# Tommachilez/improving-learned-index

Measured on AMD Instinct MI355X. Metric: docs/sec encoded + queries/sec@top-1000, MS MARCO passage, 1/2/4/8 MI355X, higher is better.
Workload: dtype bf16x3

## Files before the change

improving-learned-index_amd/csrc/enc_attn.hip:

```cpp
#include <hip/hip_runtime.h>

#include <algorithm>
#include <cstdlib>
#include <type_traits>

#include "di_common.h"
#include "enc_common.h"

namespace di {

constexpr int ATT_D = 64;
constexpr int QT = 4;

__host__ __device__ __forceinline__ int vt_base(int doc, int tok0) { return 32 * (doc + (tok0 >> 5)); }

template <typename T>
struct AttnOps;
template <>
struct AttnOps<bf16> {
    static constexpr int KC = 32;
    static constexpr int EPC = 8;
};
template <>
struct AttnOps<float> {
    static constexpr int KC = 16;
    static constexpr int EPC = 4;
};

__device__ __forceinline__ void mma_chunk(const uint4 &a, const uint4 &b, f32x4 &acc, bf16) {
    bf16x8 av, bv;
    __builtin_memcpy(&av, &a, 16);
    __builtin_memcpy(&bv, &b, 16);
    acc = __builtin_amdgcn_mfma_f32_16x16x32_bf16(av, bv, acc, 0, 0, 0);
}
__device__ __forceinline__ void mma_chunk(const uint4 &a, const uint4 &b, f32x4 &acc, float) {
    acc = __builtin_amdgcn_mfma_f32_16x16x4f32(__uint_as_float(a.x), __uint_as_float(b.x), acc,
                                               0, 0, 0);
    acc = __builtin_amdgcn_mfma_f32_16x16x4f32(__uint_as_float(a.y), __uint_as_float(b.y), acc,
                                               0, 0, 0);
    acc = __builtin_amdgcn_mfma_f32_16x16x4f32(__uint_as_float(a.z), __uint_as_float(b.z), acc,
                                               0, 0, 0);
    acc = __builtin_amdgcn_mfma_f32_16x16x4f32(__uint_as_float(a.w), __uint_as_float(b.w), acc,
                                               0, 0, 0);
}

template <typename T>
__global__ void __launch_bounds__(64)
attention_kernel(const T *__restrict__ qk, const T *__restrict__ vt,
                 const int32_t *__restrict__ cu_seqlens, int H, int ld_v, int n_qb, int n_heads,
                 int n_pairs, T *__restrict__ ctx, bf16 *__restrict__ ctx_split) {
    constexpr int KC = AttnOps<T>::KC, EPC = AttnOps<T>::EPC;
    constexpr int NCH = ATT_D / KC;
    const int id = blockIdx.x, x = id & 7, j = id >> 3;
    const int pair = (j / n_qb) * 8 + x;
    const int qb = j % n_qb;
    if (pair >= n_pairs) return;
    const int doc = pair / n_heads, h = pair % n_heads;
    const int lane = threadIdx.x;
    const int g = lane >> 4, c = lane & 15;
    const int tok0 = cu_seqlens[doc], n = cu_seqlens[doc + 1] - tok0;
// ... 112 lines not shown
                    acc = __builtin_amdgcn_mfma_f32_16x16x4f32(__uint_as_float(a0.w), s[0][3], acc, 0, 0, 0);
                    acc = __builtin_amdgcn_mfma_f32_16x16x4f32(__uint_as_float(a1.x), s[1][0], acc, 0, 0, 0);
                    acc = __builtin_amdgcn_mfma_f32_16x16x4f32(__uint_as_float(a1.y), s[1][1], acc, 0, 0, 0);
                    acc = __builtin_amdgcn_mfma_f32_16x16x4f32(__uint_as_float(a1.z), s[1][2], acc, 0, 0, 0);
                    acc = __builtin_amdgcn_mfma_f32_16x16x4f32(__uint_as_float(a1.w), s[1][3], acc, 0, 0, 0);
                    o[qt][dt] = acc;
                }
            }
        }
    }
#pragma unroll
    for (int qt = 0; qt < QT; ++qt) {
        float l = lsum[qt];
        l += __shfl_xor(l, 16, 64);
        l += __shfl_xor(l, 32, 64);
        const float inv = 1.0f / l;
        const int q = q_base + 16 * qt + c;
        if (q < n && ctx_split) {
            bf16 *out = ctx_split + (int64_t)(tok0 + q) * 2 * H;
#pragma unroll
            for (int dt = 0; dt < 4; ++dt) {
                bf16x4 hv, lv;
#pragma unroll
                for (int r = 0; r < 4; ++r) hv[r] = split_hi(o[qt][dt][r] * inv), lv[r] = split_lo(o[qt][dt][r] * inv);
                const int64_t sc0 = split_col(h * ATT_D + dt * 16 + 4 * g);
                *reinterpret_cast<bf16x4 *>(out + sc0) = hv;
                *reinterpret_cast<bf16x4 *>(out + sc0 + 32) = lv;
            }
        } else if (q < n) {
            T *out = ctx + (int64_t)(tok0 + q) * H + h * ATT_D + 4 * g;
#pragma unroll
            for (int dt = 0; dt < 4; ++dt) {
                if constexpr (sizeof(T) == 2) {
                    bf16x4 v;
#pragma unroll
                    for (int r = 0; r < 4; ++r) v[r] = (bf16)(o[qt][dt][r] * inv);
                    *reinterpret_cast<bf16x4 *>(out + dt * 16) = v;
                } else {
                    *reinterpret_cast<float4 *>(out + dt * 16) =
                        make_float4(o[qt][dt][0] * inv, o[qt][dt][1] * inv, o[qt][dt][2] * inv,
                                    o[qt][dt][3] * inv);
                }
            }
        }
    }
}

constexpr int AX_WAVES = 8, AX_QT = 2;
__device__ __forceinline__ int ax_swz(int r) { return ((r & 3) << 1) | (r & 8); }
constexpr int AX_KC = 64, AX_IMG = AX_KC * 256, AX_LDS = 4 * AX_IMG;
constexpr int AX_QTB = 4096;
constexpr int ax_lds(int nw, int qtn, int kc = AX_KC) { return 4 * kc * 256 + nw * qtn * AX_QTB; }

template <bool BAL, bool LAZY, bool PIPE = false, int NW = AX_WAVES, int QTN = AX_QT,
          int KC = AX_KC>
__global__ void __launch_bounds__(64 * NW) __attribute__((amdgpu_waves_per_eu(2)))
attention_x3_kernel(const bf16 *__restrict__ qkv, const int32_t *__restrict__ cu_seqlens, int H,
                    int n_heads, int n_pairs, bf16 *__restrict__ ctx_split,
                    const int32_t *__restrict__ qsel, const int32_t *__restrict__ cu_qsel,
                    int abl) {
    extern __shared__ __attribute__((aligned(16))) unsigned char lds[];
    typedef __attribute__((address_space(3))) void lds_void;
    const int tid = threadIdx.x, lane = tid & 63;
    const int wave = __builtin_amdgcn_readfirstlane(tid >> 6);
    const int g = lane >> 4, c = lane & 15;
    const int64_t ld = 6 * (int64_t)H;
    const uint32_t lds_base =
        (uint32_t)(uintptr_t)((__attribute__((address_space(3))) unsigned char *)lds);
    const float sc = 0.125f * 1.4426950408889634f;
    constexpr int PASS_Q = NW * QTN * 16;
    static_assert(QTN == 2 || QTN == 3, "two or three query tiles per wave");
    constexpr int IMG = KC * 256, KVL = 4 * IMG;

    struct Unit {
        int pair, pass, tok0, n, h, q0, nq;
    };
    auto make_unit = [&](int pr, int pass, Unit &u) {
        const int doc = pr / n_heads;
        u.pair = pr;
        u.pass = pass;
        u.h = pr % n_heads;
        u.tok0 = cu_seqlens[doc];
        u.n = cu_seqlens[doc + 1] - u.tok0;
        u.q0 = qsel ? cu_qsel[doc] : u.tok0;
        u.nq = qsel ? cu_qsel[doc + 1] - u.q0 : u.n;
    };
    auto next_unit = [&](const Unit &u, Unit &nu) {
        if ((u.pass + 1) * PASS_Q < u.nq && !(abl & 16)) {
            nu = u;
            nu.pass = u.pass + 1;
            return true;
        }
        for (int pr = u.pair + (int)gridDim.x; pr < n_pairs; pr += (int)gridDim.x) {
            make_unit(pr, 0, nu);
            if (nu.n > 0 && nu.nq > 0) return true;
        }
        return false;
    };
    constexpr int RPW = KC / NW;
    const int sr = RPW * wave + (lane >> 4);
    auto stage = [&](const Unit &u, int ci, int b) {
        const bf16 *kg = qkv + split_col(H + u.h * ATT_D);
        const bf16 *vg = qkv + split_col(2 * H + u.h * ATT_D);
#pragma unroll
        for (int pc = 0; pc < RPW / 4; ++pc) {
            const int rl = sr + 4 * pc;
            const int row = u.tok0 + min(ci * KC + rl, u.n - 1);
            const int j = (lane & 15) ^ ax_swz(rl);
            const int dst = b * IMG + (RPW * wave + 4 * pc) * 256;
            __builtin_amdgcn_global_load_lds((const void *)(kg + row * ld + j * 8),
                                             (lds_void *)(lds + dst), 16, 0, 0);
            __builtin_amdgcn_global_load_lds((const void *)(vg + row * ld + j * 8),
                                             (lds_void *)(lds + 2 * IMG + dst), 16, 0, 0);
        }
    };
    auto qtile = [&](int qt) { return BAL ? 16 * (wave + NW * qt) : wave * (QTN * 16) + 16 * qt; };
    auto dma_q = [&](const Unit &u) {
        const bf16 *qbase = qkv + split_col(u.h * ATT_D) + 8 * g;
#pragma unroll
        for (int qt = 0; qt < QTN; ++qt) {
            const int qi = min(u.pass * PASS_Q + qtile(qt) + c, u.nq - 1);
            const int qloc = qsel ? min(max(qsel[u.q0 + qi], 0), u.n - 1) : qi;
            const int qrow = u.tok0 + qloc;
#pragma unroll
            for (int ch = 0; ch < 2; ++ch) {
                const bf16 *src = qbase + qrow * ld + ch * 64;
                const int dst = KVL + wave * (QTN * AX_QTB) + (qt * 2 + ch) * 2048;
                __builtin_amdgcn_global_load_lds((const void *)src, (lds_void *)(lds + dst), 16, 0, 0);
                __builtin_amdgcn_global_load_lds((const void *)(src + 32),
                                                 (lds_void *)(lds + dst + 1024), 16, 0, 0);
            }
        }
    };
    constexpr int AX_HALF = 1024;
    uint32_t ka[2][2];
#pragma unroll
    for (int ch = 0; ch < 2; ++ch)
#pragma unroll
        for (int pt = 0; pt < 2; ++pt) {
            const int r = 8 * (c >> 2) + (c & 3), j = ch * 8 + pt * 4 + g;
            ka[ch][pt] = lds_base + r * 256 + ((j ^ ax_swz(r)) << 4);
        }
    uint32_t va[4][2];
#pragma unroll
    for (int dt = 0; dt < 4; ++dt)
#pragma unroll
        for (int pt = 0; pt < 2; ++pt) {
            const int q = c >> 2, pp = c & 3;
            const int r = 8 * g + q;
            const int j = (dt >> 1) * 8 + pt * 4 + 2 * (dt & 1) + (pp >> 1);
            va[dt][pt] = lds_base + 2 * IMG + r * 256 + ((j ^ ax_swz(r)) << 4) + 8 * (pp & 1);
        }

    Unit cu;
    {
        int pr = blockIdx.x;
        for (; pr < n_pairs; pr += (int)gridDim.x) {
            make_unit(pr, 0, cu);
            if (cu.n > 0 && cu.nq > 0) break;
        }
        if (pr >= n_pairs) return;
    }
    bf16x8 qh[QTN][2], ql[QTN][2];
    const uint32_t qa = lds_base + KVL + wave * (QTN * AX_QTB) + lane * 16;
    auto read_q = [&]() {
        uint4 q4[8];
        asm volatile(
            "ds_read_b128 %0, %8 offset:0"
            "\n\tds_read_b128 %1, %8 offset:1024"
            "\n\tds_read_b128 %2, %8 offset:2048"
            "\n\tds_read_b128 %3, %8 offset:3072"
            "\n\tds_read_b128 %4, %8 offset:4096"
            "\n\tds_read_b128 %5, %8 offset:5120"
            "\n\tds_read_b128 %6, %8 offset:6144"
            "\n\tds_read_b128 %7, %8 offset:7168"
            "\n\ts_waitcnt lgkmcnt(0)"
            : "=&v"(q4[0]), "=&v"(q4[1]), "=&v"(q4[2]), "=&v"(q4[3]), "=&v"(q4[4]),
              "=&v"(q4[5]), "=&v"(q4[6]), "=&v"(q4[7])
            : "v"(qa)
            : "memory");
#pragma unroll
        for (int qt = 0; qt < 2; ++qt)
#pragma unroll
            for (int ch = 0; ch < 2; ++ch) {
                __builtin_memcpy(&qh[qt][ch], &q4[(qt * 2 + ch) * 2], 16);
                __builtin_memcpy(&ql[qt][ch], &q4[(qt * 2 + ch) * 2 + 1], 16);
            }
        if constexpr (QTN == 3) {
            uint4 q5[4];
            asm volatile(
                "ds_read_b128 %0, %4 offset:8192"
                "\n\tds_read_b128 %1, %4 offset:9216"
                "\n\tds_read_b128 %2, %4 offset:10240"
                "\n\tds_read_b128 %3, %4 offset:11264"
                "\n\ts_waitcnt lgkmcnt(0)"
                : "=&v"(q5[0]), "=&v"(q5[1]), "=&v"(q5[2]), "=&v"(q5[3])
                : "v"(qa)
                : "memory");
#pragma unroll
            for (int ch = 0; ch < 2; ++ch) {
                __builtin_memcpy(&qh[2][ch], &q5[ch * 2], 16);
                __builtin_memcpy(&ql[2][ch], &q5[ch * 2 + 1], 16);
            }
        }
    };
    stage(cu, 0, 0);
    dma_q(cu);
    int b = 0;
    for (;;) {
        const int n = cu.n, h = cu.h, q0 = cu.q0, nq = cu.nq;
        const int q_pass = cu.pass * PASS_Q;
        const bool has_q = q_pass + qtile(0) < nq;
        const bool two = BAL ? q_pass + qtile(1) < nq : has_q;
        const bool three = QTN == 3 && (BAL ? q_pass + qtile(2) < nq : has_q);
// ... 352 lines not shown
                            vfr[dt][p == 1], p == 2 ? pl[qt] : ph[qt], o[qt][dt], 0, 0, 0);
            }
            }
            };
            chunk(nqt_outer);
        };
        const int n_whole = n / KC;
        int ci = 0;
        for (; ci < n_whole; ++ci, b ^= 1) one_chunk(ci, std::true_type{});
        if (ci < n_chunks) {
            one_chunk(ci, std::false_type{});
            b ^= 1;
        }
        };
        if (!has_q) {
            for (int ci = 0; ci < n_chunks; ++ci, b ^= 1)
                if (ci > 0) stage_step(ci);
        } else if (three) {
            if constexpr (QTN == 3) chunk_loop(std::integral_constant<int, 3>{});
        } else if (two) {
            chunk_loop(std::integral_constant<int, 2>{});
        } else {
            chunk_loop(std::integral_constant<int, 1>{});
        }
        if (has_q) {
#pragma unroll
            for (int qt = 0; qt < QTN; ++qt) {
                float l = lsum[qt];
                l += __shfl_xor(l, 16, 64);
                l += __shfl_xor(l, 32, 64);
                const float inv = 1.0f / l;
                const int q = q_pass + qtile(qt) + c;
                if (q < nq) {
                    bf16 *out = ctx_split + (int64_t)(q0 + q) * 2 * H;
#pragma unroll
                    for (int dt = 0; dt < 4; ++dt) {
                        bf16x4 hv, lv;
#pragma unroll
                        for (int r = 0; r < 4; ++r) {
                            const float y = o[qt][dt][r] * inv;
                            hv[r] = split_hi(y);
                            lv[r] = split_lo(y);
                        }
                        const int64_t sc0 = split_col(h * ATT_D + dt * 16 + 4 * g);
                        *reinterpret_cast<bf16x4 *>(out + sc0) = hv;
                        *reinterpret_cast<bf16x4 *>(out + sc0 + 32) = lv;
                    }
                }
            }
        }
        if (!more) break;
        cu = nu;
    }
#undef AX_READ_K
#undef AX_READ_VW
#undef AX_SEL
}

void launch_attention_x3(const bf16 *qkv, const int32_t *cu_seqlens, int n_docs, int H,
                         bf16 *ctx_split, hipStream_t s, const int32_t *qsel,
                         const int32_t *cu_qsel) {
    DI_REQUIRE(H % ATT_D == 0, DI_EINVAL, "hidden %d is not a multiple of the head dim 64", H);
    if (n_docs == 0) return;
    const int n_heads = H / ATT_D;
    const int64_t n_pairs = (int64_t)n_docs * n_heads;
    DI_REQUIRE(n_pairs < (1ll << 31), DI_ERANGE, "attention grid too large");
    static const int variant = [] {
        const char *e = getenv("DI_ATTN_X3");
        return e ? atoi(e) & 252 : 92;
    }();

    static const int abl = [] {
        const char *e = getenv("DI_ATTN_X3_ABLATE");
        return e ? atoi(e) : 0;
    }();
#define AX_LAUNCH(BL, LZ, PP, NW, QN, KC)                                                      \
    do {                                                                                       \
        DI_HIP(hipFuncSetAttribute((const void *)attention_x3_kernel<BL, LZ, PP, NW, QN, KC>,  \
                                   hipFuncAttributeMaxDynamicSharedMemorySize,                 \
                                   ax_lds(NW, QN, KC)));                                       \
        hipLaunchKernelGGL((attention_x3_kernel<BL, LZ, PP, NW, QN, KC>),                      \
                           dim3((int)std::min<int64_t>(                                        \
                               n_pairs, (int64_t)n_cu() * (160 * 1024 / ax_lds(NW, QN, KC)))), \
                           dim3(64 * NW), ax_lds(NW, QN, KC), s, qkv, cu_seqlens, H, n_heads,  \
                           (int)n_pairs, ctx_split, qsel, cu_qsel, abl);                       \
    } while (0)
    static const int pruned_variant = [] {
        const char *e = getenv("DI_ATTN_X3_PRUNED");
        return e ? atoi(e) : 1;
    }();
    if (qsel && pruned_variant == 1 && variant == 92) {
        AX_LAUNCH(true, true, true, 4, 3, 32);
        check_launch("attention_x3");
        return;
    }
    switch (variant) {
    case 12: AX_LAUNCH(true, true, false, AX_WAVES, AX_QT, AX_KC); break;
    case 28: AX_LAUNCH(true, true, true, AX_WAVES, AX_QT, AX_KC); break;
    case 60: AX_LAUNCH(true, true, true, 4, AX_QT, AX_KC); break;
    case 92: AX_LAUNCH(true, true, true, AX_WAVES, 3, AX_KC); break;
    case 220: AX_LAUNCH(true, true, true, 4, 3, 32); break;
    default: AX_LAUNCH(false, false, false, AX_WAVES, AX_QT, AX_KC); break;
    }
#undef AX_LAUNCH
    check_launch("attention_x3");
}

__device__ __forceinline__ bool softmax_need(const f32x4 (&s)[2], float lim) {
    bool need = false;
#pragma unroll
    for (int t = 0; t < 2; ++t)
#pragma unroll
        for (int r = 0; r < 4; ++r) need |= s[t][r] > lim;
    return need;
}
__device__ __forceinline__ void softmax_rescale(const f32x4 (&s)[2], float lim, float &m,
                                                float &msc, f32x4 (&o)[4], f32x4 &l) {
    constexpr float sc = 0.125f * 1.4426950408889634f;
    float cmax = fmaxf(fmaxf(fmaxf(s[0][0], s[0][1]), fmaxf(s[0][2], s[0][3])),
                       fmaxf(fmaxf(s[1][0], s[1][1]), fmaxf(s[1][2], s[1][3])));
    const auto p16 = __builtin_amdgcn_permlane16_swap(__float_as_uint(cmax),
                                                      __float_as_uint(cmax), false, false);
    cmax = fmaxf(__uint_as_float(p16[0]), __uint_as_float(p16[1]));
    const auto p32 = __builtin_amdgcn_permlane32_swap(__float_as_uint(cmax),
                                                      __float_as_uint(cmax), false, false);
    cmax = fmaxf(__uint_as_float(p32[0]), __uint_as_float(p32[1]));
    const float m_new = cmax > lim ? fmaxf(m, cmax) : m;
    const float alpha = exp2f((m - m_new) * sc);
    m = m_new;
    msc = m_new * sc;
    l *= alpha;
#pragma unroll
    for (int dt = 0; dt < 4; ++dt) o[dt] *= alpha;
}
__device__ __forceinline__ void softmax_p(const f32x4 (&s)[2], float msc, bf16x8 &pb) {
    constexpr float sc = 0.125f * 1.4426950408889634f;
#pragma unroll
    for (int r = 0; r < 4; ++r) {
        pb[r] = (bf16)__builtin_amdgcn_exp2f(fmaf(s[0][r], sc, -msc));
        pb[4 + r] = (bf16)__builtin_amdgcn_exp2f(fmaf(s[1][r], sc, -msc));
    }
}

constexpr int ATT3_WAVES = 8;
template <bool DB>
struct Att3 {
    static constexpr int ROWS = DB ? 320 : 512;
    static constexpr int BUF = 2 * ROWS * 128;
    static constexpr int LDS = DB ? 2 * BUF : BUF;
};

__device__ __forceinline__ int att3_swz(int r) { return (r & 7) ^ ((r >> 1) & 4); }

template <int K, int N, class F>
__device__ __forceinline__ void att3_chunks(F &f) {
    if constexpr (K < N) {
        if (f(std::integral_constant<int, K>{})) return;
        att3_chunks<K + 1, N>(f);
// ... 432 lines not shown
```

improving-learned-index_amd/csrc/enc_handle.h:

```cpp
#pragma once

#include <memory>
#include <vector>

#include "di_common.h"
#include "pair_order.h"

namespace di {

struct Layer {
    DevBuf w_qkv, b_qkv, w_o, b_o, ln1_g, ln1_b, w_i, b_i, w_out, b_out, ln2_g, ln2_b;
    DevBuf s_qkv, c_qkv, s_i, c_i;
};

struct PairRun {
    const int32_t *tt, *ct;
    const int64_t *cu_sq;
    int max_len;
};

}

struct di_encoder {
    di_encoder_cfg cfg{};
    int device = 0;
    hipStream_t stream = nullptr;
    bool own_stream = false;
    size_t esz = 2;
    bool split = false;
    di::DevBuf word, pos, type0, emb_g, emb_b, head_w;
    float head_b = 0.f;
    std::vector<std::unique_ptr<di::Layer>> layers;
    di::DevBuf X, qk, vt, vcol, ctx, pre, X1, Hff, impact, ids, cu, tt, cut, err;
    bool folded = false;
    di::DevBuf stats1, stats2, head_wg;
    di::DevBuf rln1, rln2;
    float head_sw = 0.f, head_cw = 0.f;
    int64_t cap_tokens = 0;
    int64_t cap_rows = 0;
    int cap_docs = 0;
    int ld_v = 0;
    bool has_pair = false;
    di::DevBuf pair_w, Mx, uv, cu_sq, cup;
    float pair_w0 = 0.f, pair_b = 0.f;
    const di::PairRun *pair_run = nullptr;
    di::DevBuf ent_single, ent_pair, ent_pos;
    di::PairOrderWs order;
    di::DevBuf pinfo;
    di::Timer timer;
};

namespace di {

void ensure_workspace(di_encoder *e, int64_t M, int n_docs, int64_t n_terms);

}
```

improving-learned-index_amd/csrc/encoder.hip:

```cpp
#include <hip/hip_runtime.h>

#include <cstdlib>
#include <type_traits>

#include <cmath>
#include <cstring>
#include <memory>
#include <string>
#include <unordered_map>
#include <vector>

#include "di_common.h"
#include "enc_common.h"
#include "enc_handle.h"

namespace di {

template <typename T>
void launch_gemm(int epi, const GemmArgs &g, hipStream_t s);
template <typename T>
void launch_attention(const T *qk, const T *vt, const int32_t *cu_seqlens, int n_docs,
                      int max_len, int H, int ld_v, T *ctx, hipStream_t s,
                      bf16 *ctx_split = nullptr);
void launch_gemm256(int epi, const GemmArgs &g, hipStream_t s);
void launch_attention_x3(const bf16 *qkv, const int32_t *cu_seqlens, int n_docs, int H,
                         bf16 *ctx_split, hipStream_t s, const int32_t *qsel = nullptr,
                         const int32_t *cu_qsel = nullptr);
void launch_scatter_term_rows(const bf16 *Xg, const int32_t *cu_seq, const int32_t *cu_terms,
                              const int32_t *term_tok, int n_docs, int W, int64_t ld, bf16 *X,
                              hipStream_t s);
void launch_embed_ln_split(const int32_t *ids, const int32_t *cu, int n_docs, int M, int H,
                           const float *word, const float *pos, const float *type0,
                           const float *gamma, const float *beta, float eps, int pos_offset,
                           int vocab, int max_pos, bf16 *out, int32_t *err, hipStream_t s);
void launch_ln_split(const float *pre, int M, int H, const float *gamma, const float *beta,
                     float eps, bf16 *out, const float *head_w, float head_b, int act,
                     float *impact, hipStream_t s);
template <typename T>
void launch_embed_ln(const int32_t *ids, const int32_t *cu, int n_docs, int M, int H,
                     const T *word, const T *pos, const T *type0, const float *gamma,
                     const float *beta, float eps, int pos_offset, int vocab, int max_pos, T *out,
                     int32_t *err, hipStream_t s);
template <typename T>
void launch_ln(const T *pre, int M, int H, const float *gamma, const float *beta, float eps,
               T *out, const float *head_w, float head_b, int act, float *impact, hipStream_t s);
void launch_vt_cols(const int32_t *cu, int n_docs, int M, int32_t *vcol, hipStream_t s);
bool attention_v3_ok(int max_len, int H);
void launch_head_from_stats(const float4 *st, int ld, int n_part, int M, int H, float eps,
                            float sw, float cw, int act, float *impact, hipStream_t s);
void launch_row_ln(const float4 *st, int ld, int n_part, int M, int H, float eps, float2 *out,
                   hipStream_t s);
int gemm_stats_cols();
void launch_attention_v3(const bf16 *qkv, const int32_t *cu_seqlens, int n_docs, int max_len,
                         int H, bf16 *ctx, hipStream_t s, const int32_t *qsel = nullptr,
                         const int32_t *cu_qsel = nullptr);
void launch_gather_term_rows(const bf16 *X, const float2 *rl, const int32_t *cu_seq,
                             const int32_t *cu_terms, const int32_t *term_tok, int n_docs, int H,
                             bf16 *Xg, float2 *rlg, hipStream_t s);
int vt_ld(int64_t M, int n_docs);
void launch_gather_terms(const float *impact, const int32_t *cu_seq, const int32_t *cu_terms,
                         int n_docs, const int32_t *term_tok, int n_terms, int do_round,
                         float *out, int32_t *err, hipStream_t s);

size_t pair_attn_lds_bytes(int max_len);
void launch_pair_prep(const int32_t *cu_seq, const int32_t *cu_terms, const int32_t *term_tok,
                      const int64_t *cu_pairs, int n_docs, int64_t n_terms, int64_t n_pairs,
                      int max_len, int64_t *cu_sq, int32_t *err, hipStream_t s);
void launch_pair_attn(const void *qk, bool split, const int32_t *cu_seq, const int32_t *cu_terms,
                      const int32_t *term_tok, const int64_t *cu_sq, int n_docs, int max_len,
                      int H, float *Mx, const int32_t *err, hipStream_t s);
void launch_pair_score(const void *src, int src_mode, const int32_t *cu_seq,
                       const int32_t *cu_terms, const int32_t *term_tok,
                       const int64_t *cu_pairs, const int64_t *cu_sq, int n_docs,
                       int64_t n_terms, int64_t n_pairs, int H, const float *gamma,
                       const float *beta, float eps, const float *w, float w0, float bias,
                       const float *Mx, float2 *uv, int do_round, float *out_pair,
                       float *out_attn, const int32_t *err, hipStream_t s);

}

// ... 122 lines not shown
            uint16_t *o = &h[(size_t)(r * 2 * K)];
            for (int k = 0; k < K; ++k) {
                const float w = p->at(i * K + k);
                const uint16_t hi = f32_to_bf16_bits(w);
                const uint16_t lo = f32_to_bf16_bits(w - bf16_bits_to_f32(hi));
                o[split_col(k)] = hi;
                o[split_col(k) + 32] = lo;
            }
        }
    }
    dst.reserve(h.size() * 2);
    DI_HIP(hipMemcpy(dst.p, h.data(), h.size() * 2, hipMemcpyHostToDevice));
}

}

void di::ensure_workspace(di_encoder *e, int64_t M, int n_docs, int64_t n_terms) {
    const int H = e->cfg.hidden, F = e->cfg.intermediate;
    if (M > e->cap_tokens || n_docs > e->cap_docs) {
        int64_t cap = std::max<int64_t>(std::max<int64_t>(M, e->cap_tokens), 256);
        const int capd = std::max(std::max(n_docs, e->cap_docs), 16);
        const size_t es = e->esz;
        const int64_t capr = (cap + 255) / 256 * 256;
        e->X.reserve(capr * H * es);
        e->X1.reserve(capr * H * es);
        e->ctx.reserve(capr * H * es);
        e->qk.reserve(cap * 3 * H * es);
        e->Hff.reserve(capr * std::max(F, H) * es);
        e->pre.reserve(cap * H * es);
        e->impact.reserve(cap * 4);
        e->ids.reserve(cap * 4);
        const size_t vt_bytes = e->split ? 0 : (size_t)H * vt_ld(cap, capd) * es;
        if (!e->split) e->vcol.reserve(cap * 4);
        if (vt_bytes > e->vt.bytes) {
            e->vt.reserve(vt_bytes);
            DI_HIP(hipMemset(e->vt.p, 0, vt_bytes));
        }
        if (e->folded) {
            const size_t sb = (size_t)(H / 128) * capr * 16;
            e->stats1.reserve(sb);
            e->stats2.reserve(sb);
            e->rln1.reserve((size_t)capr * 8);
            e->rln2.reserve((size_t)capr * 8);
        }
        e->cap_tokens = cap;
        e->cap_rows = capr;
        e->cap_docs = capd;
    }
    e->ld_v = vt_ld(M, n_docs);
    e->cu.reserve((size_t)(n_docs + 1) * 4);
    e->cut.reserve((size_t)(n_docs + 1) * 4);
    e->tt.reserve((size_t)std::max<int64_t>(n_terms, 1) * 4);
    e->err.reserve(16);
    if (e->has_pair) {
        e->uv.reserve((size_t)std::max<int64_t>(n_terms, 1) * 8);
        e->cu_sq.reserve((size_t)(n_docs + 1) * 8);
        e->cup.reserve((size_t)(n_docs + 1) * 8);
        e->ent_single.reserve((size_t)std::max<int64_t>(n_terms, 1) * 4);
        e->ent_pos.reserve((size_t)std::max<int64_t>(n_terms, 1) * 4);
        e->order.reserve_docs(n_docs);
    }
}

namespace {

void pair_attn_layer(di_encoder *e, const int32_t *d_cu, int n_docs, bool timing,
                     hipStream_t s) {
    const PairRun *r = e->pair_run;
    if (!r) return;
    TimedLaunch tl(e->timer, timing, "pair_attn", s);
    launch_pair_attn(e->qk.p, e->split, d_cu, r->ct, r->tt, r->cu_sq, n_docs, r->max_len,
                     e->cfg.hidden, e->Mx.as<float>(), e->err.as<int32_t>(), s);
}

template <typename T>
void forward(di_encoder *e, const int32_t *d_ids, const int32_t *d_cu, int n_docs, int64_t M,
             int max_len, bool timing, hipStream_t s) {
    const auto &c = e->cfg;
    const int H = c.hidden, F = c.intermediate;
    const int pos_offset = (c.variant == DI_VARIANT_XLMR) ? c.pad_id + 1 : 0;
    T *X = e->X.as<T>(), *X1 = e->X1.as<T>();
    {
        TimedLaunch tl(e->timer, timing, "embed_ln", s);
        launch_embed_ln<T>(d_ids, d_cu, n_docs, (int)M, H, e->word.as<T>(), e->pos.as<T>(),
                           e->type0.as<T>(), e->emb_g.as<float>(), e->emb_b.as<float>(),
                           c.layer_norm_eps, pos_offset, c.vocab_size, c.max_positions, X,
                           e->err.as<int32_t>(), s);
    }
    const bool use_v3 = std::is_same<T, bf16>::value && attention_v3_ok(max_len, H);
    if (!use_v3) launch_vt_cols(d_cu, n_docs, (int)M, e->vcol.as<int32_t>(), s);
    for (size_t l = 0; l < e->layers.size(); ++l) {
        Layer &L = *e->layers[l];
        const bool last = l + 1 == e->layers.size();
        GemmArgs g{};
        g.M = (int)M;
        g.a_rows = e->cap_rows;
        g.hidden = H;
        if (use_v3) {
            g.A = X;
            g.B = L.w_qkv.p;
            g.bias = L.b_qkv.as<float>();
            g.out = e->qk.p;
            g.N = 3 * H;
            g.K = H;
            g.ld_out = 3 * H;
            {
// ... 147 lines not shown
            TimedLaunch tl(e->timer, timing, "gather_rows", s);
            Xr = e->Hff.as<bf16>();
            launch_gather_term_rows(X, P ? rl2 : nullptr, d_cu, d_ct, d_tt, n_docs, H * W2, Xr,
                                    rl1, s);
            rl2r = rl1;
        };
        const bool qc = prune && sp;
        if (qc) gather_rows();
        GemmArgs g = base();
        g.A = X;
        g.B = L.w_qkv.p;
        g.bias = L.b_qkv.as<float>();
        g.out = e->qk.p;
        g.N = 3 * H;
        g.K = H;
        g.ld_out = 3 * H * W2;
        if (P) {
            g.row_ln = rl2;
            g.col_s = L.s_qkv.as<float>();
            g.col_c = L.c_qkv.as<float>();
        }
        {
            TimedLaunch tl(e->timer, timing, "gemm_qkv", s);
            if (!qc) {
                gemm(P ? EPI_FOLD : EPI_BIAS, g);
            } else {
                GemmArgs gk = g;
                gk.B = static_cast<const bf16 *>(L.w_qkv.p) + (int64_t)H * 2 * H;
                gk.bias = L.b_qkv.as<float>() + H;
                if (P) {
                    gk.col_s = L.s_qkv.as<float>() + H;
                    gk.col_c = L.c_qkv.as<float>() + H;
                }
                gk.out = e->qk.as<bf16>() + 2 * H;
                gk.N = 2 * H;
                gemm(P ? EPI_FOLD : EPI_BIAS, gk);
                GemmArgs gq = g;
                gq.A = Xr;
                gq.M = (int)n_terms;
                gq.N = H;
                gq.out = e->ctx.p;
                gq.ld_out = 2 * H;
                gq.row_ln = P ? rl1 : nullptr;
                gemm(P ? EPI_FOLD : EPI_BIAS, gq);
                launch_scatter_term_rows(e->ctx.as<bf16>(), d_cu, d_ct, d_tt, n_docs, 2 * H,
                                         6 * (int64_t)H, e->qk.as<bf16>(), s);
            }
        }
        if (sp) pair_attn_layer(e, d_cu, n_docs, timing, s);
        {
            TimedLaunch tl(e->timer, timing, "attention", s);
            if (sp)
                launch_attention_x3(e->qk.as<bf16>(), d_cu, n_docs, H, e->ctx.as<bf16>(), s,
                                    prune ? d_tt : nullptr, prune ? d_ct : nullptr);
            else
                launch_attention_v3(e->qk.as<bf16>(), d_cu, n_docs, max_len, H,
                                    e->ctx.as<bf16>(), s, prune ? d_tt : nullptr,
                                    prune ? d_ct : nullptr);
        }
        if (prune && !qc) gather_rows();
        auto base_r = [&]() {
            GemmArgs gr = base();
            gr.M = (int)Mr;
            return gr;
        };
        g = base_r();
        g.A = e->ctx.p;
        g.B = L.w_o.p;
        g.bias = L.b_o.as<float>();
        g.resid = Xr;
        g.out = X1;
        g.N = H;
        g.K = H;
        g.ld_out = H * W2;
        g.stats_out = st1;
        if (P) {
            g.row_ln = rl2r;
            g.res_gamma = P->ln2_g.as<float>();
            g.res_beta = P->ln2_b.as<float>();
        }
        {
            TimedLaunch tl(e->timer, timing, "gemm_o", s);
            gemm(EPI_RESID_STATS, g);
        }
        {
            TimedLaunch tl(e->timer, timing, "row_ln", s);
            launch_row_ln(st1, ld, n_part, (int)Mr, H, c.layer_norm_eps, rl1, s);
        }
        g = base_r();
        g.A = X1;
        g.B = L.w_i.p;
        g.out = e->Hff.p;
        g.N = F;
        g.K = H;
        g.ld_out = F * W2;
        g.row_ln = rl1;
        g.col_s = L.s_i.as<float>();
        g.col_c = L.c_i.as<float>();
        {
            TimedLaunch tl(e->timer, timing, "gemm_ffn1", s);
            gemm(EPI_FOLD_GELU, g);
        }
        g = base_r();
        g.A = e->Hff.p;
        g.B = L.w_out.p;
        g.bias = L.b_out.as<float>();
        g.resid = X1;
// ... 21 lines not shown
        launch_head_from_stats(st2, ld, n_part, (int)(d_tt ? n_terms : M), H, c.layer_norm_eps,
                               e->head_sw,
                               e->head_cw, c.activation, e->impact.as<float>(), s);
    }
}

void forward_split(di_encoder *e, const int32_t *d_ids, const int32_t *d_cu, int n_docs,
                   int64_t M, int max_len, bool timing, hipStream_t s,
                   const int32_t *d_tt = nullptr, const int32_t *d_ct = nullptr,
                   int64_t n_terms = 0) {
    const auto &c = e->cfg;
    const int H = c.hidden, F = c.intermediate;
    const int pos_offset = (c.variant == DI_VARIANT_XLMR) ? c.pad_id + 1 : 0;
    bf16 *X = e->X.as<bf16>(), *X1 = e->X1.as<bf16>(), *ctx = e->ctx.as<bf16>();
    float *pre = e->pre.as<float>();
    {
        TimedLaunch tl(e->timer, timing, "embed_ln", s);
        launch_embed_ln_split(d_ids, d_cu, n_docs, (int)M, H, e->word.as<float>(),
                              e->pos.as<float>(), e->type0.as<float>(), e->emb_g.as<float>(),
                              e->emb_b.as<float>(), c.layer_norm_eps, pos_offset, c.vocab_size,
                              c.max_positions, X, e->err.as<int32_t>(), s);
    }
    auto base = [&]() {
        GemmArgs g{};
        g.M = (int)M;
        g.a_rows = e->cap_rows;
        g.hidden = H;
        g.tune_gm = 8;
        g.split = 1;
        return g;
    };
    for (size_t l = 0; l < e->layers.size(); ++l) {
        Layer &L = *e->layers[l];
        const bool last = l + 1 == e->layers.size();
        GemmArgs g = base();
        g.A = X;
        g.B = L.w_qkv.p;
        g.bias = L.b_qkv.as<float>();
        g.out = e->qk.p;
        g.N = 3 * H;
        g.K = H;
        g.ld_out = 6 * H;
        {
            TimedLaunch tl(e->timer, timing, "gemm_qkv", s);
            launch_gemm256(EPI_BIAS, g, s);
        }
        const bool prune = last && d_tt != nullptr;
        const int64_t Mr = prune ? n_terms : M;
        bf16 *Xr = X;
        pair_attn_layer(e, d_cu, n_docs, timing, s);
        {
            TimedLaunch tl(e->timer, timing, "attention", s);
            launch_attention_x3(e->qk.as<bf16>(), d_cu, n_docs, H, ctx, s,
                                prune ? d_tt : nullptr, prune ? d_ct : nullptr);
        }
        if (prune) {
            TimedLaunch tl(e->timer, timing, "gather_rows", s);
            Xr = e->Hff.as<bf16>();
            launch_gather_term_rows(X, nullptr, d_cu, d_ct, d_tt, n_docs, 2 * H, Xr, nullptr, s);
        }
        auto base_r = [&]() {
            GemmArgs gr = base();
            gr.M = (int)Mr;
            return gr;
        };
        g = base_r();
        g.A = ctx;
        g.B = L.w_o.p;
        g.bias = L.b_o.as<float>();
        g.resid = Xr;
        g.out = pre;
        g.N = H;
        g.K = H;
        g.ld_out = H;
        {
            TimedLaunch tl(e->timer, timing, "gemm_o", s);
            launch_gemm256(EPI_BIAS_RESID, g, s);
        }
        {
            TimedLaunch tl(e->timer, timing, "ln", s);
            launch_ln_split(pre, (int)Mr, H, L.ln1_g.as<float>(), L.ln1_b.as<float>(),
                            c.layer_norm_eps, X1, nullptr, 0.f, c.activation, nullptr, s);
        }
        g = base_r();
        g.A = X1;
        g.B = L.w_i.p;
        g.bias = L.b_i.as<float>();
        g.out = e->Hff.p;
        g.N = F;
        g.K = H;
        g.ld_out = 2 * F;
        {
            TimedLaunch tl(e->timer, timing, "gemm_ffn1", s);
            launch_gemm256(EPI_BIAS_GELU, g, s);
        }
        g = base_r();
        g.A = e->Hff.p;
        g.B = L.w_out.p;
        g.bias = L.b_out.as<float>();
        g.resid = X1;
        g.out = pre;
        g.N = H;
        g.K = F;
        g.ld_out = H;
        g.tune_gm = 4;
        {
            TimedLaunch tl(e->timer, timing, "gemm_ffn2", s);
// ... 65 lines not shown
                mx_need += T * T;
            }
            n_pairs = pc->cu_pairs[n_docs];
        }
    } else if (pc) {
        DI_REQUIRE(n_terms >= 0 && n_terms <= n_tokens && n_pairs >= 0, DI_EINVAL,
                   "n_terms=%lld n_pairs=%lld", (long long)n_terms, (long long)n_pairs);
        mx_need = n_terms * std::min<int64_t>(n_terms, max_len);
    }
    DI_REQUIRE(n_tokens >= 0 && n_tokens < (1ll << 31), DI_ERANGE, "n_tokens=%lld",
               (long long)n_tokens);
    DI_REQUIRE(max_len <= e->cfg.max_positions, DI_ERANGE,
               "a document has %d tokens > max_positions %d", max_len,
               e->cfg.max_positions);
    if (pc && pc->n_terms_out) *pc->n_terms_out = n_terms, *pc->n_pairs_out = n_pairs;
    if (n_docs == 0) return;
    ensure_workspace(e, n_tokens, n_docs, n_terms);
    float *out_pair = pc ? pc->out_pair : nullptr;
    if (pc && pc->dev_out) {
        e->ent_pair.reserve((size_t)std::max<int64_t>(n_pairs, 1) * 4);
        out = e->ent_single.as<float>();
        out_pair = e->ent_pair.as<float>();
    }
    const int32_t *d_ids = stage_in(tok_ids, (size_t)n_tokens, dev, e->ids, s);
    const int32_t *d_cu = stage_in(cu_seqlens, (size_t)n_docs + 1, dev, e->cu, s);
    DI_HIP(hipMemsetAsync(e->err.p, 0, 4, s));
    const int32_t *d_tt = nullptr, *d_cut = nullptr;
    if (!token_out) {
        d_tt = stage_in(term_tok, (size_t)n_terms, dev, e->tt, s);
        d_cut = stage_in(cu_terms, (size_t)n_docs + 1, dev, e->cut, s);
    }
    PairRun run{};
    struct RunScope {
        di_encoder *e;
        ~RunScope() { e->pair_run = nullptr; }
    } run_scope{e};
    const int64_t *d_cup = nullptr;
    if (pc) {
        DI_REQUIRE(pair_attn_lds_bytes(max_len) <= 160 * 1024, DI_ERANGE,
                   "pairwise: a document of %d tokens exceeds the LDS panel", max_len);
        DI_REQUIRE(mx_need <= (1ll << 32), DI_ERANGE,
                   "pairwise: %lld term-pair slots in one batch (limit 2^32)",
                   (long long)mx_need);
        e->Mx.reserve((size_t)std::max<int64_t>(mx_need, 1) * 4);
        d_cup = stage_in(pc->cu_pairs, (size_t)n_docs + 1, dev, e->cup, s);
        {
            TimedLaunch tl(e->timer, timing, "pair_prep", s);
            if (mx_need) DI_HIP(hipMemsetAsync(e->Mx.p, 0, (size_t)mx_need * 4, s));
            launch_pair_prep(d_cu, d_cut, d_tt, d_cup, n_docs, n_terms, n_pairs, max_len,
                             e->cu_sq.as<int64_t>(), e->err.as<int32_t>(), s);
        }
        run = PairRun{d_tt, d_cut, e->cu_sq.as<int64_t>(), max_len};
        if (n_pairs > 0) e->pair_run = &run;
    }
    const bool prune = !token_out && (e->split || (e->esz == 2 && e->folded)) &&
                       n_terms <= n_tokens;
    if (n_tokens > 0) {
        if (e->split && !e->folded)
            forward_split(e, d_ids, d_cu, n_docs, n_tokens, max_len, timing, s,
                          prune ? d_tt : nullptr, prune ? d_cut : nullptr, n_terms);
        else if (e->split)
            forward_folded(e, d_ids, d_cu, n_docs, n_tokens, max_len, timing, s,
                           prune ? d_tt : nullptr, prune ? d_cut : nullptr, n_terms);
        else if (e->esz == 2)
            if (e->folded)
                forward_folded(e, d_ids, d_cu, n_docs, n_tokens, max_len, timing, s,
                               prune ? d_tt : nullptr, prune ? d_cut : nullptr, n_terms);
            else
                forward<bf16>(e, d_ids, d_cu, n_docs, n_tokens, max_len, timing, s);
        else
            forward<float>(e, d_ids, d_cu, n_docs, n_tokens, max_len, timing, s);
    }
    float *d_out = out;
    DevBuf tmp;
    if (token_out) {
        if (dev)
            DI_HIP(hipMemcpyAsync(out, e->impact.p, (size_t)n_tokens * 4,
                                  hipMemcpyDeviceToDevice, s));
        else
            DI_HIP(hipMemcpyAsync(out, e->impact.p, (size_t)n_tokens * 4,
                                  hipMemcpyDeviceToHost, s));
    } else {
        if (!dev_out) {
            tmp.reserve((size_t)std::max<int64_t>(n_terms, 1) * 4);
            d_out = tmp.as<float>();
        }
        {
            TimedLaunch tl(e->timer, timing, "gather_terms", s);
            launch_gather_terms(e->impact.as<float>(), d_cu, d_cut, n_docs, d_tt,
                                (int)n_terms,
                                ((flags & DI_F_ROUND3) ? 1 : 0) | (prune && n_tokens > 0 ? 2 : 0),
                                d_out, e->err.as<int32_t>(), s);
        }
        if (!dev_out && n_terms)
            DI_HIP(hipMemcpyAsync(out, d_out, (size_t)n_terms * 4, hipMemcpyDeviceToHost,
                                  s));
    }
    DevBuf tmp_pair, tmp_attn;
    if (pc && n_pairs > 0) {
        float *d_pair = out_pair, *d_attn = pc->out_attn;
        if (!dev_out) {
            tmp_pair.reserve((size_t)n_pairs * 4);
            d_pair = tmp_pair.as<float>();
            if (pc->out_attn) {
                tmp_attn.reserve((size_t)n_pairs * 4);
                d_attn = tmp_attn.as<float>();
// ... 321 lines not shown
```

Measured before the change: 12270.

## Sort docs by length for attention scheduling and split long/short launches

Adds a single-block GPU kernel that counting-sorts documents by descending length and writes boundaries for long (>192 tokens) and short groups. The attention_x3 kernel now walks this order in a serpentine block assignment, which balances per-block work and shrinks tail imbalance. By default it also runs two launches, a large 8-wave configuration for long docs and a smaller 4-wave/KC=32 one for short docs. The cost is an extra serial sort kernel per batch and a second attention launch. The grid size now uses the queried LDS-per-CU instead of a hardcoded 160KB.

```diff
diff --git a/improving-learned-index_amd/csrc/enc_attn.hip b/improving-learned-index_amd/csrc/enc_attn.hip
--- a/improving-learned-index_amd/csrc/enc_attn.hip
+++ b/improving-learned-index_amd/csrc/enc_attn.hip
@@ -1,11 +1,14 @@
 #include <hip/hip_runtime.h>
 
 #include <algorithm>
+#include <atomic>
 #include <cstdlib>
 #include <type_traits>
+#include <vector>
 
 #include "di_common.h"
 #include "enc_common.h"
+#include "enc_handle.h"
 
 namespace di {
 
@@ -224,18 +227,28 @@
 constexpr int AX_QTB = 4096;
 constexpr int ax_lds(int nw, int qtn, int kc = AX_KC) { return 4 * kc * 256 + nw * qtn * AX_QTB; }
 
+#ifdef DI_ATTN_STAMP
+__device__ unsigned long long ax_stamp[2][1024];
+#endif
+
 template <bool BAL, bool LAZY, bool PIPE = false, int NW = AX_WAVES, int QTN = AX_QT,
           int KC = AX_KC>
 __global__ void __launch_bounds__(64 * NW) __attribute__((amdgpu_waves_per_eu(2)))
 attention_x3_kernel(const bf16 *__restrict__ qkv, const int32_t *__restrict__ cu_seqlens, int H,
                     int n_heads, int n_pairs, bf16 *__restrict__ ctx_split,
                     const int32_t *__restrict__ qsel, const int32_t *__restrict__ cu_qsel,
+                    const int32_t *__restrict__ q_order, const int32_t *__restrict__ q_range,
                     int abl) {
     extern __shared__ __attribute__((aligned(16))) unsigned char lds[];
     typedef __attribute__((address_space(3))) void lds_void;
     const int tid = threadIdx.x, lane = tid & 63;
     const int wave = __builtin_amdgcn_readfirstlane(tid >> 6);
     const int g = lane >> 4, c = lane & 15;
+#ifdef DI_ATTN_STAMP
+    if (lane == 0)
+        atomicMin(&ax_stamp[0][blockIdx.x], (unsigned long long)__builtin_amdgcn_s_memrealtime());
+    __builtin_amdgcn_s_waitcnt(0xC07F);
+#endif
     const int64_t ld = 6 * (int64_t)H;
     const uint32_t lds_base =
         (uint32_t)(uintptr_t)((__attribute__((address_space(3))) unsigned char *)lds);
@@ -245,17 +258,24 @@
     constexpr int IMG = KC * 256, KVL = 4 * IMG;
 
     struct Unit {
-        int pair, pass, tok0, n, h, q0, nq;
+        int r, pass, tok0, n, h, q0, nq;
     };
-    auto make_unit = [&](int pr, int pass, Unit &u) {
-        const int doc = pr / n_heads;
-        u.pair = pr;
-        u.pass = pass;
-        u.h = pr % n_heads;
+    const int q_lo = q_order ? q_range[0] : 0;
+    const int n_units = q_order ? (q_range[1] - q_lo) * n_heads : n_pairs;
+    auto make_unit = [&](int r, Unit &u) {
+        const int gs = (int)gridDim.x, bx = (int)blockIdx.x;
+        const int64_t i = (int64_t)r * gs + ((q_order && (r & 1)) ? gs - 1 - bx : bx);
+        if (i >= n_units) return false;
+        const int di = (int)i / n_heads;
+        const int doc = q_order ? q_order[q_lo + di] : di;
+        u.r = r;
+        u.pass = 0;
+        u.h = (int)i - di * n_heads;
         u.tok0 = cu_seqlens[doc];
         u.n = cu_seqlens[doc + 1] - u.tok0;
         u.q0 = qsel ? cu_qsel[doc] : u.tok0;
         u.nq = qsel ? cu_qsel[doc + 1] - u.q0 : u.n;
+        return true;
     };
     auto next_unit = [&](const Unit &u, Unit &nu) {
         if ((u.pass + 1) * PASS_Q < u.nq && !(abl & 16)) {
@@ -263,10 +283,8 @@
             nu.pass = u.pass + 1;
             return true;
         }
-        for (int pr = u.pair + (int)gridDim.x; pr < n_pairs; pr += (int)gridDim.x) {
-            make_unit(pr, 0, nu);
+        for (int r = u.r + 1; make_unit(r, nu); ++r)
             if (nu.n > 0 && nu.nq > 0) return true;
-        }
         return false;
     };
     constexpr int RPW = KC / NW;
@@ -325,13 +343,9 @@
         }
 
     Unit cu;
-    {
-        int pr = blockIdx.x;
-        for (; pr < n_pairs; pr += (int)gridDim.x) {
-            make_unit(pr, 0, cu);
-            if (cu.n > 0 && cu.nq > 0) break;
-        }
-        if (pr >= n_pairs) return;
+    for (int r = 0;; ++r) {
+        if (!make_unit(r, cu)) return;
+        if (cu.n > 0 && cu.nq > 0) break;
     }
     bf16x8 qh[QTN][2], ql[QTN][2];
     const uint32_t qa = lds_base + KVL + wave * (QTN * AX_QTB) + lane * 16;
@@ -790,14 +804,169 @@
         if (!more) break;
         cu = nu;
     }
+#ifdef DI_ATTN_STAMP
+    if (lane == 0)
+        atomicMax(&ax_stamp[1][blockIdx.x], (unsigned long long)__builtin_amdgcn_s_memrealtime());
+#endif
 #undef AX_READ_K
 #undef AX_READ_VW
 #undef AX_SEL
 }
 
+constexpr int AQ_THREADS = 1024, AQ_TILE = 4096;
+__global__ void __launch_bounds__(AQ_THREADS)
+attn_order_kernel(const int32_t *__restrict__ cu_seqlens, int n_docs, int max_len, int long_len,
+                  int32_t *__restrict__ order, int32_t *__restrict__ ctl) {
+    extern __shared__ int32_t aq_lds[];
+    int32_t *start = aq_lds, *tile = aq_lds + (max_len + 1);
+    const int tid = threadIdx.x;
+    auto len_of = [&](int d) {
+        return min(max(cu_seqlens[d + 1] - cu_seqlens[d], 0), max_len);
+    };
+    for (int b = tid; b <= max_len; b += AQ_THREADS) start[b] = 0;
+    __syncthreads();
+    for (int d = tid; d < n_docs; d += AQ_THREADS) atomicAdd(&start[len_of(d)], 1);
+    __syncthreads();
+    if (tid == 0) {
+        int acc = 0, n_long = 0;
+        for (int b = max_len; b >= 0; --b) {
+            const int cnt = start[b];
+            start[b] = acc;
+            acc += cnt;
+            if (b == long_len + 1) n_long = acc;
+        }
+        ctl[0] = 0;
+        ctl[1] = n_long;
+        ctl[2] = n_docs;
+        ctl[3] = 0;
+        ctl[4] = n_docs;
+    }
+    __syncthreads();
+    for (int t0 = 0; t0 < n_docs; t0 += AQ_TILE) {
+        const int nt = min(AQ_TILE, n_docs - t0);
+        for (int i = tid; i < nt; i += AQ_THREADS) tile[i] = len_of(t0 + i);
+        __syncthreads();
+        for (int b = tid; b <= max_len; b += AQ_THREADS) {
+            int pos = start[b];
+            for (int i = 0; i < nt; ++i)
+                if (tile[i] == b) order[pos++] = t0 + i;
+            start[b] = pos;
+        }
+        __syncthreads();
+    }
+}
+
+bool attn_order_ok(int max_positions) {
+    return max_positions >= 0 && (size_t)(max_positions + 1 + AQ_TILE) * 4 <= 64 * 1024;
+}
+
+void launch_attn_order(const int32_t *cu_seqlens, int n_docs, int max_positions, int32_t *order,
+                       int32_t *ctl, hipStream_t s) {
+    DI_REQUIRE(attn_order_ok(max_positions), DI_ERANGE, "attention order: max_positions %d",
+               max_positions);
+    hipLaunchKernelGGL(attn_order_kernel, dim3(1), dim3(AQ_THREADS),
+                       (size_t)(max_positions + 1 + AQ_TILE) * 4, s, cu_seqlens, n_docs,
+                       max_positions, AQ_LONG_LEN, order, ctl);
+    check_launch("attn_order");
+}
+
+int attn_queue_mode() {
+    static const int mode = [] {
+        const char *e = getenv("DI_ATTN_X3_QUEUE");
+        return e ? atoi(e) : 2;
+    }();
+    return mode;
+}
+
+namespace {
+
+void ax_lds_limits(int &per_cu, int &per_wg) {
+    int dev = 0, cu = 0, wg = 0;
+    DI_HIP(hipGetDevice(&dev));
+    DI_HIP(hipDeviceGetAttribute(&wg, hipDeviceAttributeMaxSharedMemoryPerBlock, dev));
+    (void)hipDeviceGetAttribute(&cu, hipDeviceAttributeMaxSharedMemoryPerMultiprocessor, dev);
+    per_wg = wg;
+    per_cu = std::max(cu, wg);
+}
+
+struct AxArgs {
+    const bf16 *qkv;
+    const int32_t *cu_seqlens;
+    int H, n_heads;
+    int64_t n_pairs;
+    bf16 *ctx_split;
+    const int32_t *qsel, *cu_qsel, *q_order, *q_range;
+    int abl;
+    hipStream_t s;
+};
+
+template <bool BL, bool LZ, bool PP, int NW, int QN, int KC>
+void ax_launch(const AxArgs &a) {
+    constexpr int LDS = ax_lds(NW, QN, KC);
+    const auto kern = attention_x3_kernel<BL, LZ, PP, NW, QN, KC>;
+    int dev = 0, per_cu = 0, per_wg = 0;
+    DI_HIP(hipGetDevice(&dev));
+    ax_lds_limits(per_cu, per_wg);
+    DI_REQUIRE(LDS <= per_wg, DI_ERANGE, "attention_x3: %d bytes of LDS, the device gives %d",
+               LDS, per_wg);
+    static std::atomic<uint64_t> set_on{0};
+    const uint64_t bit = dev < 64 ? 1ull << dev : 0;
+    if (!(set_on.load(std::memory_order_acquire) & bit)) {
+        DI_HIP(hipFuncSetAttribute((const void *)kern,
+                                   hipFuncAttributeMaxDynamicSharedMemorySize, LDS));
+        set_on.fetch_or(bit, std::memory_order_release);
+    }
+    const int grid = (int)std::min<int64_t>(a.n_pairs, (int64_t)n_cu() * (per_cu / LDS));
+#ifdef DI_ATTN_STAMP
+    unsigned long long *st = nullptr;
+    DI_HIP(hipGetSymbolAddress((void **)&st, HIP_SYMBOL(ax_stamp)));
+    DI_HIP(hipMemsetAsync(st, 0xFF, 1024 * 8, a.s));
+    DI_HIP(hipMemsetAsync(st + 1024, 0, 1024 * 8, a.s));
+#endif
+    hipLaunchKernelGGL(kern, dim3(grid), dim3(64 * NW), LDS, a.s, a.qkv, a.cu_seqlens, a.H,
+                       a.n_heads, (int)a.n_pairs, a.ctx_split, a.qsel, a.cu_qsel, a.q_order,
+                       a.q_range, a.abl);
+    check_launch("attention_x3");
+#ifdef DI_ATTN_STAMP
+    static int n_launch = 0;
+    static const int from = getenv("DI_ATTN_STAMP_FROM") ? atoi(getenv("DI_ATTN_STAMP_FROM")) : 0;
+    static const int cnt = getenv("DI_ATTN_STAMP_COUNT") ? atoi(getenv("DI_ATTN_STAMP_COUNT")) : 0;
+    if (n_launch >= from && n_launch < from + cnt && grid <= 1024) {
+        static unsigned long long h[2][1024];
+        DI_HIP(hipStreamSynchronize(a.s));
+        DI_HIP(hipMemcpy(h, st, sizeof h, hipMemcpyDeviceToHost));
+        unsigned long long t0 = ~0ull, t1 = 0;
+        double sum = 0;
+        int nb = 0;
+        std::vector<unsigned long long> ends;
+        for (int i = 0; i < grid; ++i)
+            if (h[1][i]) {
+                t0 = std::min(t0, h[0][i]);
+                t1 = std::max(t1, h[1][i]);
+                ends.push_back(h[1][i]);
+                ++nb;
+            }
+        if (nb) {
+            std::sort(ends.begin(), ends.end());
+            for (auto e : ends) sum += (double)(e - t0);
+            const double span = (double)(t1 - t0), mean = sum / nb;
+            fprintf(stderr,
+                    "ax_stamp launch %d NW=%d qsel=%d list=%d grid=%d busy=%d span_us=%.1f "
+                    "mean_end=%.4f first_end=%.4f median_end=%.4f p90_end=%.4f tail=%.4f\n",
+                    n_launch, NW, a.qsel != nullptr, a.q_order != nullptr, grid, nb, span * 0.01,
+                    mean / span, (ends.front() - t0) / span, (ends[nb / 2] - t0) / span,
+                    (ends[nb * 9 / 10] - t0) / span, 1.0 - mean / span);
+        }
+    }
+    ++n_launch;
+#endif
+}
+
+}
+
 void launch_attention_x3(const bf16 *qkv, const int32_t *cu_seqlens, int n_docs, int H,
                          bf16 *ctx_split, hipStream_t s, const int32_t *qsel,
-                         const int32_t *cu_qsel) {
+                         const int32_t *cu_qsel, const AttnQueue *q) {
     DI_REQUIRE(H % ATT_D == 0, DI_EINVAL, "hidden %d is not a multiple of the head dim 64", H);
     if (n_docs == 0) return;
     const int n_heads = H / ATT_D;
@@ -812,36 +981,32 @@
         const char *e = getenv("DI_ATTN_X3_ABLATE");
         return e ? atoi(e) : 0;
     }();
-#define AX_LAUNCH(BL, LZ, PP, NW, QN, KC)                                                      \
-    do {                                                                                       \
-        DI_HIP(hipFuncSetAttribute((const void *)attention_x3_kernel<BL, LZ, PP, NW, QN, KC>,  \
-                                   hipFuncAttributeMaxDynamicSharedMemorySize,                 \
-                                   ax_lds(NW, QN, KC)));                                       \
-        hipLaunchKernelGGL((attention_x3_kernel<BL, LZ, PP, NW, QN, KC>),                      \
-                           dim3((int)std::min<int64_t>(                                        \
-                               n_pairs, (int64_t)n_cu() * (160 * 1024 / ax_lds(NW, QN, KC)))), \
-                           dim3(64 * NW), ax_lds(NW, QN, KC), s, qkv, cu_seqlens, H, n_heads,  \
-                           (int)n_pairs, ctx_split, qsel, cu_qsel, abl);                       \
-    } while (0)
+    if (q && !q->order) q = nullptr;
+    AxArgs a{qkv, cu_seqlens, H, n_heads, n_pairs, ctx_split, qsel, cu_qsel,
+             q ? q->order : nullptr, q ? q->ctl + AQ_ALL : nullptr, abl, s};
     static const int pruned_variant = [] {
         const char *e = getenv("DI_ATTN_X3_PRUNED");
         return e ? atoi(e) : 1;
     }();
     if (qsel && pruned_variant == 1 && variant == 92) {
-        AX_LAUNCH(true, true, true, 4, 3, 32);
-        check_launch("attention_x3");
+        ax_launch<true, true, true, 4, 3, 32>(a);
         return;
     }
+    if (q && q->two_forms && !qsel && variant == 92) {
+        a.q_range = q->ctl + AQ_LONG;
+        ax_launch<true, true, true, AX_WAVES, 3, AX_KC>(a);
+        a.q_range = q->ctl + AQ_SHORT;
+        ax_launch<true, true, true, 4, 3, 32>(a);
+        return;
+    }
     switch (variant) {
-    case 12: AX_LAUNCH(true, true, false, AX_WAVES, AX_QT, AX_KC); break;
-    case 28: AX_LAUNCH(true, true, true, AX_WAVES, AX_QT, AX_KC); break;
-    case 60: AX_LAUNCH(true, true, true, 4, AX_QT, AX_KC); break;
-    case 92: AX_LAUNCH(true, true, true, AX_WAVES, 3, AX_KC); break;
-    case 220: AX_LAUNCH(true, true, true, 4, 3, 32); break;
-    default: AX_LAUNCH(false, false, false, AX_WAVES, AX_QT, AX_KC); break;
-    }
-#undef AX_LAUNCH
-    check_launch("attention_x3");
+    case 12: ax_launch<true, true, false, AX_WAVES, AX_QT, AX_KC>(a); break;
+    case 28: ax_launch<true, true, true, AX_WAVES, AX_QT, AX_KC>(a); break;
+    case 60: ax_launch<true, true, true, 4, AX_QT, AX_KC>(a); break;
+    case 92: ax_launch<true, true, true, AX_WAVES, 3, AX_KC>(a); break;
+    case 220: ax_launch<true, true, true, 4, 3, 32>(a); break;
+    default: ax_launch<false, false, false, AX_WAVES, AX_QT, AX_KC>(a); break;
+    }
 }
 
 __device__ __forceinline__ bool softmax_need(const f32x4 (&s)[2], float lim) {
diff --git a/improving-learned-index_amd/csrc/enc_handle.h b/improving-learned-index_amd/csrc/enc_handle.h
--- a/improving-learned-index_amd/csrc/enc_handle.h
+++ b/improving-learned-index_amd/csrc/enc_handle.h
@@ -18,6 +18,18 @@
     const int64_t *cu_sq;
     int max_len;
 };
+
+struct AttnQueue {
+    const int32_t *order = nullptr;
+    const int32_t *ctl = nullptr;
+    bool two_forms = false;
+};
+constexpr int AQ_CTL = 5, AQ_LONG = 0, AQ_SHORT = 1, AQ_ALL = 3;
+constexpr int AQ_LONG_LEN = 192;
+int attn_queue_mode();
+bool attn_order_ok(int max_positions);
+void launch_attn_order(const int32_t *cu_seqlens, int n_docs, int max_positions, int32_t *order,
+                       int32_t *ctl, hipStream_t s);
 
 }
 
@@ -46,6 +58,8 @@
     const di::PairRun *pair_run = nullptr;
     di::DevBuf ent_single, ent_pair, ent_pos;
     di::PairOrderWs order;
+    di::DevBuf aq_order, aq_ctl;
+    di::AttnQueue aq;
     di::DevBuf pinfo;
     di::Timer timer;
 };
diff --git a/improving-learned-index_amd/csrc/encoder.hip b/improving-learned-index_amd/csrc/encoder.hip
--- a/improving-learned-index_amd/csrc/encoder.hip
+++ b/improving-learned-index_amd/csrc/encoder.hip
@@ -25,7 +25,7 @@
 void launch_gemm256(int epi, const GemmArgs &g, hipStream_t s);
 void launch_attention_x3(const bf16 *qkv, const int32_t *cu_seqlens, int n_docs, int H,
                          bf16 *ctx_split, hipStream_t s, const int32_t *qsel = nullptr,
-                         const int32_t *cu_qsel = nullptr);
+                         const int32_t *cu_qsel = nullptr, const AttnQueue *q = nullptr);
 void launch_scatter_term_rows(const bf16 *Xg, const int32_t *cu_seq, const int32_t *cu_terms,
                               const int32_t *term_tok, int n_docs, int W, int64_t ld, bf16 *X,
                               hipStream_t s);
@@ -254,6 +254,10 @@
     e->cut.reserve((size_t)(n_docs + 1) * 4);
     e->tt.reserve((size_t)std::max<int64_t>(n_terms, 1) * 4);
     e->err.reserve(16);
+    if (e->split) {
+        e->aq_order.reserve((size_t)std::max(e->cap_docs, n_docs) * 4);
+        e->aq_ctl.reserve(AQ_CTL * 4);
+    }
     if (e->has_pair) {
         e->uv.reserve((size_t)std::max<int64_t>(n_terms, 1) * 8);
         e->cu_sq.reserve((size_t)(n_docs + 1) * 8);
@@ -507,7 +511,7 @@
             TimedLaunch tl(e->timer, timing, "attention", s);
             if (sp)
                 launch_attention_x3(e->qk.as<bf16>(), d_cu, n_docs, H, e->ctx.as<bf16>(), s,
-                                    prune ? d_tt : nullptr, prune ? d_ct : nullptr);
+                                    prune ? d_tt : nullptr, prune ? d_ct : nullptr, &e->aq);
             else
                 launch_attention_v3(e->qk.as<bf16>(), d_cu, n_docs, max_len, H,
                                     e->ctx.as<bf16>(), s, prune ? d_tt : nullptr,
@@ -635,7 +639,7 @@
         {
             TimedLaunch tl(e->timer, timing, "attention", s);
             launch_attention_x3(e->qk.as<bf16>(), d_cu, n_docs, H, ctx, s,
-                                prune ? d_tt : nullptr, prune ? d_ct : nullptr);
+                                prune ? d_tt : nullptr, prune ? d_ct : nullptr, &e->aq);
         }
         if (prune) {
             TimedLaunch tl(e->timer, timing, "gather_rows", s);
@@ -807,6 +811,16 @@
         }
         run = PairRun{d_tt, d_cut, e->cu_sq.as<int64_t>(), max_len};
         if (n_pairs > 0) e->pair_run = &run;
+    }
+    e->aq = AttnQueue{};
+    if (e->split && n_tokens > 0 && attn_queue_mode() > 0 &&
+        attn_order_ok(e->cfg.max_positions)) {
+        TimedLaunch tl(e->timer, timing, "attn_order", s);
+        launch_attn_order(d_cu, n_docs, e->cfg.max_positions, e->aq_order.as<int32_t>(),
+                          e->aq_ctl.as<int32_t>(), s);
+        e->aq.order = e->aq_order.as<int32_t>();
+        e->aq.ctl = e->aq_ctl.as<int32_t>();
+        e->aq.two_forms = attn_queue_mode() >= 2;
     }
     const bool prune = !token_out && (e->split || (e->esz == 2 && e->folded)) &&
                        n_terms <= n_tokens;
```

After: 12400, median of 6. 1.1% higher.
